# mala-lab/GGAD

Hardware: AMD Instinct MI355X
Metric: training nodes/sec (DGraph-Fin mini-batch GGAD) (higher is better)
Workload: dtype f32; 1 GPU; DGraph-Fin-size synthetic graph, mini-batch GGAD (GCN encoder); nodes=3700550, directed_entries=72953930, feat=17, emb=64, batch=150+50, graph=powerlaw(alpha=2.1,max_degree=2000), chunk_batches=150, hop2=ldsw, overlap=False, dense_cus=0, chain=0, dense_steps=XCD-resident chunk kernel: one launch per chunk on 28 CUs of one XCD, parallelism=dp1, optimizer=adam(lr=1e-3,wd=0.007), batch_streams=the reference's stream

## Files before the change

### ggad_amd/csrc/common.h

```cpp
#pragma once
#include <hip/hip_runtime.h>
#include <stdint.h>
#include <mutex>
#include "../../include/ggad_hip.h"

#define GGAD_WAVE 64
#define GGAD_MAX_D 64
#define GGAD_MAX_F 1024

void ggad_set_error(hipError_t e, const char *where);

#define GGAD_CHECK_LAUNCH(where)                 \
  do {                                           \
    hipError_t _e = hipGetLastError();           \
    if (_e != hipSuccess) {                      \
      ggad_set_error(_e, where);                 \
      return GGAD_E_LAUNCH;                      \
    }                                            \
  } while (0)

#define GGAD_REQUIRE(cond) \
  do {                     \
    if (!(cond)) return GGAD_E_INVALID; \
  } while (0)

static inline hipStream_t as_stream(ggad_stream_t s) { return reinterpret_cast<hipStream_t>(s); }

struct ggad_lds_optin {
  std::mutex mu;
  int state[64] = {};
};
template <typename... K>
static inline int ggad_lds_opt_in(ggad_lds_optin &S, int bytes, K... kernels) {
  int dev = 0;
  if (hipGetDevice(&dev) != hipSuccess || dev < 0 || dev >= 64) return 0;
  std::lock_guard<std::mutex> lock(S.mu);
  if (S.state[dev] == 0) {
    const bool ok = ((hipFuncSetAttribute((const void *)kernels, hipFuncAttributeMaxDynamicSharedMemorySize, bytes) == hipSuccess) && ...);
    (void)hipGetLastError();
    S.state[dev] = ok ? 1 : -1;
  }
  return S.state[dev];
}

__device__ __forceinline__ int lane_id() { return threadIdx.x & (GGAD_WAVE - 1); }

__device__ __forceinline__ float wave_sum(float v) {
#pragma unroll
  for (int off = 32; off >= 1; off >>= 1) v += __shfl_xor(v, off, GGAD_WAVE);
  return v;
}
__device__ __forceinline__ int wave_sum_i(int v) {
#pragma unroll
  for (int off = 32; off >= 1; off >>= 1) v += __shfl_xor(v, off, GGAD_WAVE);
  return v;
}

__device__ __forceinline__ void ggad_adam_elem(float &pi, float &mi, float &vi, float g, float wd, float sc0, float sc1) {
  float gi = fmaf(wd, pi, g);
  mi = fmaf(gi - mi, 0.1f, mi);
  vi = fmaf(0.001f * gi, gi, vi * 0.999f);
  const float denom = sqrtf(vi) / sc1 + 1e-8f;
  pi = pi - sc0 * (mi / denom);
}

__device__ __forceinline__ int lower_bound_i32(const int32_t *__restrict__ a, int lo, int hi, int key) {
  while (lo < hi) {
    int mid = (lo + hi) >> 1;
    if (a[mid] < key) lo = mid + 1; else hi = mid;
  }
  return lo;
}

__device__ __forceinline__ bool ggad_vblock(int skip, unsigned &vb, unsigned &vg) {
  const unsigned b = blockIdx.x, n = gridDim.x;
  if (skip < 0) { vb = b; vg = n; return true; }
  const unsigned sk = (unsigned)skip;
  if ((b & 7u) == sk) return false;
  vb = b - ((b >> 3) + ((b & 7u) > sk ? 1u : 0u));
  vg = n - ((n >> 3) + ((n & 7u) > sk ? 1u : 0u));
  return true;
}
static inline unsigned ggad_skip_grid(unsigned want, int skip) { return skip < 0 ? want : (unsigned)(((uint64_t)(want + 1) * 8 + 6) / 7); }

constexpr int GGAD_CTR_STRIDE = 16;
constexpr int GGAD_CTR_GROUPS = 0 * GGAD_CTR_STRIDE, GGAD_CTR_ITEMS = 1 * GGAD_CTR_STRIDE, GGAD_CTR_PART = 2 * GGAD_CTR_STRIDE,
              GGAD_CTR_CURSOR = 3 * GGAD_CTR_STRIDE, GGAD_CTR_PC = 4 * GGAD_CTR_STRIDE,
              GGAD_CTR_BIG = 5 * GGAD_CTR_STRIDE,
              GGAD_CTR_RANGE0 = 6 * GGAD_CTR_STRIDE,
              GGAD_CTR_PROF = 14 * GGAD_CTR_STRIDE;
constexpr int GGAD_RANGES = 8;
constexpr int GGAD_RANGE_DEG = 256;
constexpr int GGAD_PLAN_COUNTERS = 16 * GGAD_CTR_STRIDE;

struct ggad_plan_view {
  const int32_t *batch_ptr, *batch_ent_ptr, *nodes, *row_slot, *ent_ptr, *row_ck_ptr, *ck_rc, *ck_e0;
  int32_t n_batches, n_rows, n_ents, n_chunks;
  int32_t seg_stride;
  int64_t pair_bound;
};
int ggad_int_hop1(const ggad_mb_plan *P, const ggad_plan_view &V, int ldsw, int reset_now, hipStream_t st);
int ggad_int_global_hop2(const ggad_mb_plan *P, const ggad_plan_view &V, hipStream_t st, hipEvent_t ev0, hipEvent_t ev1);
int ggad_int_ldsw_hop2(const ggad_mb_plan *P, const ggad_plan_view &V, hipStream_t st, hipEvent_t ev0, hipEvent_t ev1);
int ggad_int_range_deg();

int ggad_int_gemm_slab(const float *A, const float *B, float *C, int M, int N, int K, int64_t lda, int64_t sbk, int64_t sbn, int64_t ldc,
                       const float *bias, int relu, hipStream_t st, const float *prelu_a = nullptr, float *C2 = nullptr, int64_t ldc2 = 0);

int64_t ggad_int_wgrad_tn_ws(int R, int m, int n);
int ggad_int_wgrad_tn(const float *P, int64_t ldp, const float *Q, int64_t ldq, int R, int m, int n, float *D, float *ws, hipStream_t st,
                      int *vpq = nullptr);

constexpr int GGAD_MB_BWD_PARTS = 256;
struct ggad_xchg_view;
bool ggad_int_wide_ok(int D, int F);
int ggad_int_wide_project(const float *params, int32_t D, int32_t F, const float *x2, const int32_t *ent_own, int32_t ent0,
                          int32_t n_ents, float *h2, ggad_stream_t stream);
int ggad_int_wide_fwd_rows(const float *params, int32_t D, int32_t F, const float *x1, const float *h2, const int32_t *ent_ptr,
                           const int32_t *ent_own, const int32_t *labels, int32_t row0, int32_t n_rows, int32_t ent0, float *h1,
                           float *nbar, float *gen, ggad_stream_t stream);
int ggad_int_wide_loss(const float *params, int32_t D, int32_t F, const float *h1, const float *nbar, const float *gen,
                       const int32_t *labels, const int32_t *pos_meta, const int32_t *row_pos, const int32_t *ent_ptr,
                       int32_t row0, int32_t n_rows, float *loss_ws, float *losses8, float *d_h1, float *d_gen, float *d_nbar,
                       float *dz, float *coef_a, float *coef_g, int32_t *step_counter, ggad_stream_t stream);
int ggad_int_wide_row_coefs(const float *params, int32_t D, int32_t F, const int32_t *labels, const int32_t *ent_ptr,
                            int32_t row0, int32_t n_rows, const float *h1, const float *gen, const float *d_h1,
                            const float *d_gen, const float *d_nbar, float *dz, float *coef_a, float *coef_g,
                            ggad_stream_t stream);
int ggad_int_wide_bwd_flat(int32_t D, int32_t F, const float *x1, const float *x2, const float *h2, const int32_t *ent_own,
                           const int32_t *ent_row, int32_t row0, int32_t n_rows, int32_t ent0, int32_t n_ents,
                           const float *coef_a, const float *coef_g, float *dw_part, ggad_stream_t stream);
int ggad_int_wide_grad_reduce(int32_t D, int32_t F, const int32_t *pos_meta, int32_t row0, int32_t n_rows, const float *losses8,
                              const float *nbar, const float *dw_part, const float *dz, const float *loss_ws, float *grads,
                              int mode, float *params, float *m, float *v, float lr, float wd, const int32_t *step_counter,
                              const ggad_xchg_view *xv, uint32_t xstep, float grad_scale, ggad_stream_t stream);
int ggad_int_wide_rows(const float *params, int32_t D, int32_t F, const float *x1, int32_t n_rows, float *out, int score,
                       ggad_stream_t stream);

constexpr int GGAD_XCHG_MAX_WORLD = 16;
struct ggad_xchg_view {
  float *peer[GGAD_XCHG_MAX_WORLD];
  int32_t rank, world;
  int64_t n;
  int32_t *err;
  unsigned long long timeout_ticks;
};
struct ggad_xchg {
  ggad_xchg_view view;
  void *local;
  size_t bytes;
  uint32_t step;
  bool opened[GGAD_XCHG_MAX_WORLD];
};
static inline size_t ggad_xchg_granules(int world, int64_t n) { return (size_t)2 * world * (size_t)n; }
```

### ggad_amd/csrc/hop2_ldsw.hip

```cpp
#include <algorithm>
#include <atomic>
#include <climits>
#include <mutex>

#include "common.h"

namespace {

#ifdef GGAD_G2_PROF
struct G2Prof { unsigned long long a[8], t; };
#define G2_ARG , G2Prof &prof
#define G2_PASS , prof
#define G2_MARK(i) do { __builtin_amdgcn_sched_barrier(0); __builtin_amdgcn_s_waitcnt(0); const unsigned long long t_ = wall_clock64(); \
                        prof.a[i] += t_ - prof.t; prof.t = t_; __builtin_amdgcn_sched_barrier(0); } while (0)
#define TC_MARK(i) do { __syncthreads(); if (threadIdx.x == 0) { const unsigned long long t_ = wall_clock64(); tcp[i] += t_ - tct; tct = t_; } } while (0)
#else
#define G2_ARG
#define G2_PASS
#define G2_MARK(i)
#define TC_MARK(i)
#endif

constexpr int SLICE = 256;
constexpr int GRP_W = 10;
constexpr int ITEM_GRAB = 4;

__global__ void __launch_bounds__(256) k_tile_offsets(const int32_t *__restrict__ rowptr, const int32_t *__restrict__ col,
                                                      int64_t n_nodes, int n_tiles, int shift, int32_t *__restrict__ off) {
  const int64_t u = (int64_t)blockIdx.x * blockDim.x + threadIdx.x;
  if (u >= n_nodes) return;
  const int s = rowptr[u], e = rowptr[u + 1];
  int32_t *o = off + u * (n_tiles + 1);
  int t = 0;
  for (int i = s; i < e; ++i) {
    const int tile = col[i] >> shift;
    while (t <= tile) { o[t] = i - s; ++t; }
  }
  while (t <= n_tiles) { o[t] = e - s; ++t; }
}

__global__ void __launch_bounds__(256) k_tm_blocksum(const int32_t *__restrict__ off, int64_t n_nodes, int n_tiles, int32_t *__restrict__ bsum) {
  __shared__ int wsum[4][64];
  const int lane = lane_id(), w = threadIdx.x >> 6;
  const int NT1 = n_tiles + 1;
  const int64_t u0 = (int64_t)blockIdx.x * 256 + 64 * w;
  for (int t0 = 0; t0 < n_tiles; t0 += 64) {
    const int t = t0 + lane;
    int acc = 0;
    if (t < n_tiles)
      for (int i = 0; i < 64 && u0 + i < n_nodes; ++i) { const int32_t *o = off + (u0 + i) * NT1 + t; acc += o[1] - o[0]; }
    wsum[w][lane] = acc;
    __syncthreads();
    if (w == 0 && t < n_tiles) bsum[(int64_t)blockIdx.x * n_tiles + t] = wsum[0][lane] + wsum[1][lane] + wsum[2][lane] + wsum[3][lane];
    __syncthreads();
  }
}

__global__ void __launch_bounds__(1024) k_tm_scan(int32_t *__restrict__ bsum, int64_t n_blocks, int n_tiles, int32_t *__restrict__ tile_base) {
  extern __shared__ int tot[];
  for (int t = threadIdx.x; t < n_tiles; t += blockDim.x) {
    int run = 0;
    int64_t b = 0;
    for (; b + 8 <= n_blocks; b += 8) {
      int v[8];
#pragma unroll
      for (int q = 0; q < 8; ++q) v[q] = bsum[(b + q) * n_tiles + t];
#pragma unroll
      for (int q = 0; q < 8; ++q) { bsum[(b + q) * n_tiles + t] = run; run += v[q]; }
    }
    for (; b < n_blocks; ++b) { const int v = bsum[b * n_tiles + t]; bsum[b * n_tiles + t] = run; run += v; }
    tot[t] = run;
  }
  __syncthreads();
  if (threadIdx.x == 0) {
    int run = 0;
    for (int t = 0; t < n_tiles; ++t) { tile_base[t] = run; run += tot[t]; }
    tile_base[n_tiles] = run;
  }
}

__global__ void __launch_bounds__(256) k_tm_fill(const int32_t *__restrict__ rowptr, const int32_t *__restrict__ col,
                                                 const int32_t *__restrict__ off, int64_t n_nodes, int n_tiles,
                                                 const int32_t *__restrict__ bsum, const int32_t *__restrict__ tile_base,
                                                 int32_t *__restrict__ tile_start, int32_t *__restrict__ col_t) {
  __shared__ int wsum[4][64];
  const int lane = lane_id(), w = threadIdx.x >> 6;
  const int NT1 = n_tiles + 1;
  const int64_t u0 = (int64_t)blockIdx.x * 256 + 64 * w;
  for (int t0 = 0; t0 <= n_tiles; t0 += 64) {
    const int t = t0 + lane;
    int acc = 0;
    if (t < n_tiles)
      for (int i = 0; i < 64 && u0 + i < n_nodes; ++i) { const int32_t *o = off + (u0 + i) * NT1 + t; acc += o[1] - o[0]; }
    wsum[w][lane] = acc;
    __syncthreads();
    if (t < n_tiles) {
      int pos = tile_base[t] + bsum[(int64_t)blockIdx.x * n_tiles + t];
      for (int ww = 0; ww < w; ++ww) pos += wsum[ww][lane];
      for (int i = 0; i < 64 && u0 + i < n_nodes; ++i) {
        const int64_t u = u0 + i;
        const int32_t *o = off + u * NT1 + t;
        const int o0 = o[0], o1 = o[1];
        tile_start[u * NT1 + t] = pos;
        const int32_t *src = col + rowptr[u] + o0;
        for (int j = 0; j < o1 - o0; ++j) col_t[pos + j] = src[j];
        pos += o1 - o0;
      }
    } else if (t == n_tiles) {
      for (int i = 0; i < 64 && u0 + i < n_nodes; ++i) tile_start[(u0 + i) * NT1 + t] = 0;
    }
    __syncthreads();
  }
}

constexpr int TW_SHIFT = 15;
constexpr int TW_TILE = 1 << TW_SHIFT;
constexpr int TW_MAXOWN = 6144;
constexpr int TW_T = 1024;
constexpr int TW_BRK = 1536;

constexpr int TT_SLAB = 128;
__global__ void __launch_bounds__(256) k_seg_transpose(const int32_t *__restrict__ tile_off, const int32_t *__restrict__ tile_start,
                                                       int n_tiles, const int32_t *__restrict__ ent_own,
                                                       const int32_t *__restrict__ ent_col, int n_ents, int64_t seg_stride,
                                                       int32_t *__restrict__ seg_t, int skip) {
  __shared__ int tl[TT_SLAB][65];
  unsigned vbx, vgx;
  if (!ggad_vblock(skip, vbx, vgx)) return;
  const int p0 = vbx * 64;
  if (p0 >= n_ents) return;
  const int lane = lane_id(), wid = threadIdx.x >> 6;
  const int NT1 = n_tiles + 1;
  int u_l = 0, own_l = 0;
  if (p0 + lane < n_ents) { own_l = ent_own[p0 + lane] == p0 + lane ? 1 : 0; u_l = own_l ? ent_col[p0 + lane] : 0; }
  for (int which = 0; which < (tile_start ? 2 : 1); ++which) {
  const int32_t *table = which ? tile_start : tile_off;
  int32_t *plane = seg_t + (which ? (int64_t)NT1 * seg_stride : 0);
  for (int t0 = 0; t0 < NT1; t0 += TT_SLAB) {
    int v0[16], v1[16];
    const int c0 = min(t0 + lane, NT1 - 1), c1 = min(t0 + 64 + lane, NT1 - 1);
#pragma unroll
    for (int jj = 0; jj < 16; ++jj) {
      const int j = wid + 4 * jj;
      const int u = __shfl(u_l, j, GGAD_WAVE);
      const int32_t *row = table + (int64_t)u * NT1;
      v0[jj] = row[c0];
      v1[jj] = row[c1];
    }
#pragma unroll
    for (int jj = 0; jj < 16; ++jj) {
      const int j = wid + 4 * jj;
      const int own = __shfl(own_l, j, GGAD_WAVE);
      if (t0 + lane < NT1) tl[lane][j] = own ? v0[jj] : 0;
      if (t0 + 64 + lane < NT1) tl[64 + lane][j] = own ? v1[jj] : 0;
    }
    __syncthreads();
    const int nt = min(TT_SLAB, NT1 - t0);
    for (int idx = threadIdx.x; idx < nt * 64; idx += 256) {
      const int tt = idx >> 6, j = idx & 63;
      if (p0 + j < n_ents) plane[(int64_t)(t0 + tt) * seg_stride + p0 + j] = tl[tt][j];
    }
    __syncthreads();
  }
  }
}

__device__ __forceinline__ int block_excl_scan_1024(int v, int *warp_buf, int *total) {
  const int lane = lane_id(), wid = threadIdx.x >> 6;
  int inc = v;
#pragma unroll
  for (int off = 1; off < 64; off <<= 1) {
    const int t = __shfl_up(inc, off, 64);
    if (lane >= off) inc += t;
  }
  if (lane == 63) warp_buf[wid] = inc;
  __syncthreads();
  int base = 0, tot = 0;
#pragma unroll
  for (int w = 0; w < 16; ++w) { const int sv = warp_buf[w]; if (w < wid) base += sv; tot += sv; }
  __syncthreads();
  *total = tot;
  return base + inc - v;
}

__global__ void __launch_bounds__(TW_T) k_tile_counts(const int32_t *__restrict__ col, const int32_t *__restrict__ seg_t,
                                                      int64_t n_cap, const int32_t *__restrict__ own_rp,
                                                      const int32_t *__restrict__ batch_ent_ptr,
                                                      const int32_t *__restrict__ pw_base, uint16_t *__restrict__ pc, int n_tiles,
                                                      int n_batches, int32_t *__restrict__ counters, int skip, int tile_major) {
  extern __shared__ __attribute__((aligned(16))) uint32_t lds_u[];
  uint32_t *cnt = lds_u;
  int *offs = reinterpret_cast<int *>(lds_u + TW_TILE / 2);
  int *segbeg = offs + TW_MAXOWN + 1;
  int *dst = segbeg + TW_MAXOWN;
  int *brk = dst + TW_MAXOWN;
  __shared__ int wbuf[16];
  unsigned vbx, vgx;
  if (!ggad_vblock(skip, vbx, vgx)) return;
  int t, b;
  const bool class_map = (tile_major & 2) != 0;
  tile_major &= 1;
  if (class_map) {
    const int nx = skip < 0 ? 8 : 7, c = (int)(blockIdx.x & 7u);
    const int ci = c - ((skip >= 0 && c > skip) ? 1 : 0);
    const unsigned j = blockIdx.x >> 3;
    const int nt_c = ci < n_tiles ? (n_tiles - ci + nx - 1) / nx : 0;
    if (j >= (unsigned)nt_c * (unsigned)n_batches) return;
    t = ci + nx * (int)(j / (unsigned)n_batches);
    b = (int)(j % (unsigned)n_batches);
  } else {
    if (vbx >= (unsigned)n_tiles * (unsigned)n_batches) return;
    t = (int)(vbx % (unsigned)n_tiles); b = (int)(vbx / (unsigned)n_tiles);
  }
  const int o0 = batch_ent_ptr[b], o1 = batch_ent_ptr[b + 1];
  const int n_own_all = o1 - o0;
  const int32_t *seg_lo = seg_t + (int64_t)t * n_cap, *seg_hi = seg_lo + n_cap;
  const int32_t *seg_st = tile_major ? seg_t + (int64_t)(n_tiles + 1 + t) * n_cap : own_rp;
#ifdef GGAD_G2_PROF
  unsigned long long tcp[8] = {0, 0, 0, 0, 0, 0, 0, 0}, tct = wall_clock64();
#endif
  for (int i = threadIdx.x; i < TW_TILE / 2; i += TW_T) cnt[i] = 0u;
  constexpr int IPT = TW_MAXOWN / TW_T;
  const int n_slabs = (n_own_all + TW_MAXOWN - 1) / TW_MAXOWN;
  const bool one_slab = n_slabs == 1;
  constexpr int CACHE_IT = 16;
  int kc[CACHE_IT], dc[CACHE_IT];
  for (int pass = 0; pass < 2; ++pass) {
    for (int slab = 0; slab < n_slabs; ++slab) {
      const int ob0 = o0 + slab * TW_MAXOWN;
      const int n_own = min(TW_MAXOWN, o1 - ob0);
      if (pass == 0 || n_slabs > 1) {
        {
          int lo_[IPT], hi_[IPT], rp_[IPT], pb_[IPT];
#pragma unroll
          for (int q = 0; q < IPT; ++q) {
            const int i = min((int)threadIdx.x + q * TW_T, n_own - 1);
            lo_[q] = seg_lo[ob0 + i]; hi_[q] = seg_hi[ob0 + i]; rp_[q] = seg_st[ob0 + i]; pb_[q] = pw_base[ob0 + i];
          }
#pragma unroll
          for (int q = 0; q < IPT; ++q) {
            const int i = (int)threadIdx.x + q * TW_T;
            if (i < n_own) { offs[i] = hi_[q] - lo_[q]; segbeg[i] = rp_[q] + (tile_major ? 0 : lo_[q]); dst[i] = pb_[q] + lo_[q]; }
          }
        }
        __syncthreads();
        TC_MARK(0);
        int len[IPT];
        int mysum = 0;
#pragma unroll
        for (int q = 0; q < IPT; ++q) {
          const int i = threadIdx.x * IPT + q;
          len[q] = (i < n_own) ? offs[i] : 0;
          mysum += len[q];
        }
        __syncthreads();
        int P0;
        int ex = block_excl_scan_1024(mysum, wbuf, &P0);
#pragma unroll
        for (int q = 0; q < IPT; ++q) {
          const int i = threadIdx.x * IPT + q;
          if (i < n_own) offs[i] = ex;
          ex += len[q];
        }
        if (threadIdx.x == 0) offs[n_own] = P0;
        __syncthreads();
        TC_MARK(1);
      }
      const int P = offs[n_own];
      if (P > 0) {
        const int s0 = 1 << (31 - __clz(n_own));
        auto locate = [&](int pp, int &own, int &j) {
          int lo = 0;
          for (int st = s0; st > 0; st >>= 1) { const int m = lo + st; lo = (offs[min(m, n_own)] <= pp) ? m : lo; }
          own = lo; j = pp - offs[lo];
        };
        const int nblk = ((P - 1) >> 6) + 1;
        const bool use_brk = nblk + 1 <= TW_BRK;
        if (use_brk && (pass == 0 || n_slabs > 1)) {
          for (int b = threadIdx.x; b <= nblk; b += TW_T) {
            int own = n_own, j = 0;
            if (b < nblk) locate(min(64 * b, P - 1), own, j);
            brk[b] = own;
          }
          __syncthreads();
        }
        auto locate4 = [&](const int (&pp)[4], int (&own)[4], int (&j)[4]) {
          int lo[4] = {0, 0, 0, 0};
          int smax = s0;
          if (use_brk) {
            smax = 0;
#pragma unroll
            for (int q = 0; q < 4; ++q) {
              const int b = pp[q] >> 6;
              lo[q] = brk[b];
              const int w = brk[b + 1] - lo[q];
              smax = max(smax, w > 0 ? 1 << (31 - __clz(w)) : 0);
            }
          }
          for (int st = smax; st > 0; st >>= 1) {
#pragma unroll
            for (int q = 0; q < 4; ++q) { const int m = lo[q] + st; lo[q] = (offs[min(m, n_own)] <= pp[q]) ? m : lo[q]; }
          }
#pragma unroll
          for (int q = 0; q < 4; ++q) { own[q] = lo[q]; j[q] = pp[q] - offs[lo[q]]; }
        };
        int p_start = 0;
        if (one_slab) {
          if (pass == 0) {
#pragma unroll
            for (int g4 = 0; g4 < CACHE_IT; g4 += 4) {
              if (g4 * TW_T < P) {
                int pp[4], own[4], j[4];
#pragma unroll
                for (int q = 0; q < 4; ++q) pp[q] = min((g4 + q) * TW_T + (int)threadIdx.x, P - 1);
                locate4(pp, own, j);
#pragma unroll
                for (int q = 0; q < 4; ++q) {
                  kc[g4 + q] = col[segbeg[own[q]] + j[q]];
                  dc[g4 + q] = dst[own[q]] + j[q];
                }
              } else {
#pragma unroll
                for (int q = 0; q < 4; ++q) { kc[g4 + q] = 0; dc[g4 + q] = 0; }
              }
            }
#pragma unroll
            for (int it = 0; it < CACHE_IT; ++it) {
              const bool on = it * TW_T + (int)threadIdx.x < P;
              const int loc = kc[it] & (TW_TILE - 1);
              if (on) atomicAdd(&cnt[loc >> 1], 1u << ((loc & 1) << 4));
              kc[it] = on ? loc : -1;
            }
          } else {
#pragma unroll
            for (int it = 0; it < CACHE_IT; ++it)
              if (kc[it] >= 0) pc[dc[it]] = (uint16_t)((cnt[kc[it] >> 1] >> ((kc[it] & 1) << 4)) & 0xFFFFu);
          }
          p_start = CACHE_IT * TW_T;
          TC_MARK(2 + 2 * pass);
        }
        for (int p0 = p_start; p0 < P; p0 += 4 * TW_T) {
          int pp[4], own[4], j[4];
#pragma unroll
          for (int q = 0; q < 4; ++q) pp[q] = min(p0 + q * TW_T + (int)threadIdx.x, P - 1);
          locate4(pp, own, j);
          int k4[4];
#pragma unroll
          for (int q = 0; q < 4; ++q) k4[q] = col[segbeg[own[q]] + j[q]];
#pragma unroll
          for (int q = 0; q < 4; ++q) {
            if (p0 + q * TW_T + (int)threadIdx.x < P) {
              const int loc = k4[q] & (TW_TILE - 1);
              if (pass == 0) atomicAdd(&cnt[loc >> 1], 1u << ((loc & 1) << 4));
              else pc[(int64_t)dst[own[q]] + j[q]] = (uint16_t)((cnt[loc >> 1] >> ((loc & 1) << 4)) & 0xFFFFu);
            }
          }
        }
        TC_MARK(3 + 2 * pass);
      }
      __syncthreads();
    }
  }
#ifdef GGAD_G2_PROF
  if (threadIdx.x == 0) {
    unsigned long long *out = reinterpret_cast<unsigned long long *>(counters + GGAD_CTR_PROF) + 8;
    for (int k = 0; k < 6; ++k) atomicAdd(out + k, tcp[k]);
    atomicAdd(out + 6, 1ull);
  }
#endif
}

template <int G, int FT>
__device__ __forceinline__ void gather_slice(const int32_t *__restrict__ col, const float *__restrict__ feat, int F_rt, int stride,
                                             int s, int n0, int n1, float inv_sr, int n_occ, const int (&pb)[8],
                                             const uint16_t *__restrict__ pc, int lane, int k_first, float (&tot)[G] G2_ARG) {
  const int F = FT ? FT : F_rt;
  const int rpi = 64 / F;
  const int g = lane / F, f = lane - g * F;
  const bool act = g < rpi;
  const int gl = act ? g : rpi - 1;
  const char *fb = reinterpret_cast<const char *>(feat);
  const uint32_t rs = (uint32_t)stride * 4u, fo = (uint32_t)f * 4u;
  auto row_elem = [&](int kk) -> float { return *reinterpret_cast<const float *>(fb + ((uint32_t)kk * rs + fo)); };
  float acc[G];
#pragma unroll
  for (int j = 0; j < G; ++j) acc[j] = 0.0f;
  const int last = max(n1 - 1, 0);
  int k_nx = k_first;
  uint32_t c_nx[G];
  {
    const int ix = min(n0 + lane, last);
#pragma unroll
    for (int j = 0; j < G; ++j) c_nx[j] = pc[pb[j] + ix];
  }
  G2_MARK(2);
  for (int blk = n0; blk < n1; blk += 64) {
    const bool mine = blk + lane < n1;
    const int k = mine ? k_nx : 0;
    const int count = min(64, n1 - blk);
    float w[G];
    if (FT != 17) {
#pragma unroll
      for (int j = 0; j < G; ++j) w[j] = (j < n_occ && mine) ? inv_sr / sqrtf((float)c_nx[j]) : 0.0f;
    }
    if (FT == 17) {
      constexpr int IT = 22;
      float x[IT];
#pragma unroll
      for (int t = 0; t < IT; ++t) {
        const int kk = __shfl(k, (t * 3 + gl) & 63, GGAD_WAVE);
        x[t] = row_elem(kk);
      }
#pragma unroll
      for (int j = 0; j < G; ++j) w[j] = (j < n_occ && mine) ? inv_sr / sqrtf((float)c_nx[j]) : 0.0f;
      {
        const int ix = min(blk + 64 + lane, last);
        k_nx = col[s + ix];
#pragma unroll
        for (int j = 0; j < G; ++j) c_nx[j] = pc[pb[j] + ix];
      }
      G2_MARK(3);
#pragma unroll
      for (int t = 0; t < IT; ++t) {
        const int src = t * 3 + g;
        const float xv = (act && src < count) ? x[t] : 0.0f;
#pragma unroll
        for (int j = 0; j < G; ++j) {
          const float ws = __shfl(w[j], src & 63, GGAD_WAVE);
          acc[j] = fmaf((src < count) ? ws : 0.0f, xv, acc[j]);
        }
      }
      G2_MARK(4);
    } else {
      const int iters = (count + rpi - 1) / rpi;
      int tt = 0;
      for (; tt + 8 <= iters; tt += 8) {
        float x[8];
#pragma unroll
        for (int q = 0; q < 8; ++q) {
          const int kk = __shfl(k, ((tt + q) * rpi + gl) & 63, GGAD_WAVE);
          x[q] = row_elem(kk);
        }
#pragma unroll
        for (int q = 0; q < 8; ++q) {
          const int src = (tt + q) * rpi + g;
          const float xv = (act && src < count) ? x[q] : 0.0f;
#pragma unroll
          for (int j = 0; j < G; ++j) {
            const float ws = __shfl(w[j], src & 63, GGAD_WAVE);
            acc[j] = fmaf((src < count) ? ws : 0.0f, xv, acc[j]);
          }
        }
      }
      for (; tt < iters; ++tt) {
        const int src = tt * rpi + g;
        const int kk = __shfl(k, (tt * rpi + gl) & 63, GGAD_WAVE);
        const float xr = row_elem(kk);
        const float xv = (act && src < count) ? xr : 0.0f;
#pragma unroll
        for (int j = 0; j < G; ++j) {
          const float ws = __shfl(w[j], src & 63, GGAD_WAVE);
          acc[j] = fmaf((src < count) ? ws : 0.0f, xv, acc[j]);
        }
      }
      const int ix = min(blk + 64 + lane, last);
      k_nx = col[s + ix];
#pragma unroll
      for (int j = 0; j < G; ++j) c_nx[j] = pc[pb[j] + ix];
    }
  }
#pragma unroll
  for (int j = 0; j < G; ++j) {
    float t = acc[j];
    for (int q = 1; q < rpi; ++q) t += __shfl(acc[j], (lane + q * F) & 63, GGAD_WAVE);
    tot[j] = t;
  }
}

constexpr int MF_WS = 68;
constexpr int MF_LDS = 8 * MF_WS + 64;
typedef float mf4 __attribute__((ext_vector_type(4)));
typedef float mf2 __attribute__((ext_vector_type(2)));
typedef int mi4 __attribute__((ext_vector_type(4)));

template <int G>
__device__ __forceinline__ void gather_slice_mfma(const int32_t *__restrict__ col, const float *__restrict__ feat, int s, int n0, int n1,
                                                  float inv_sr, int n_occ, const int (&pb)[8], const uint16_t *__restrict__ pc,
                                                  int lane, float *lw, int k_first, float (&tot)[G] G2_ARG) {
  const int a = lane & 15, g = lane >> 4;
  const char *fb = reinterpret_cast<const char *>(feat) + a * 8;
  int *lids = reinterpret_cast<int *>(lw + 8 * MF_WS);
  const int aa = a < G ? a : 0;
  mf4 acc0 = {0.0f, 0.0f, 0.0f, 0.0f}, acc1 = {0.0f, 0.0f, 0.0f, 0.0f};
  const int last = max(n1 - 1, 0);
  int k_nx = k_first;
  uint32_t c_nx[G];
  {
    const int ix = min(n0 + lane, last);
#pragma unroll
    for (int j = 0; j < G; ++j) c_nx[j] = pc[pb[j] + ix];
  }
  G2_MARK(2);
  for (int blk = n0; blk < n1; blk += 64) {
    const bool mine = blk + lane < n1;
    lids[lane] = k_nx;
    __builtin_amdgcn_fence(__ATOMIC_RELEASE, "wavefront");
    __builtin_amdgcn_wave_barrier();
    int id[16];
#pragma unroll
    for (int c = 0; c < 4; ++c) {
      const mi4 iv = *reinterpret_cast<const mi4 *>(lids + 16 * g + 4 * c);
#pragma unroll
      for (int q = 0; q < 4; ++q) id[4 * c + q] = iv[q];
    }
    mf2 x[16];
#pragma unroll
    for (int i = 0; i < 16; ++i) x[i] = *reinterpret_cast<const mf2 *>(fb + ((uint32_t)id[i] << 7));
#pragma unroll
    for (int j = 0; j < G; ++j)
      lw[j * MF_WS + lane] = (j < n_occ && mine) ? inv_sr / sqrtf((float)c_nx[j]) : 0.0f;
// ... 189 lines not shown
      int e[8], pb[8];
      int n = 0;
#pragma unroll
      for (int j = 0; j < 8; ++j) {
        e[j] = __builtin_amdgcn_readlane(rv, q * 16 + j);
        pb[j] = __builtin_amdgcn_readlane(pbv, q * 16 + j);
        n += e[j] >= 0 ? 1 : 0;
      }
      const int pbase = __builtin_amdgcn_readlane(rv, q * 16 + 8), ns = __builtin_amdgcn_readlane(rv, q * 16 + 9);
      const int sl = __builtin_amdgcn_readlane(iv, q * 16 + 1);
      int s, n0, n1, deg;
      item_span(q, s, n0, n1, deg);
      const float inv_sr = 1.0f / sqrtf((float)deg);
      const int k_first = k_ahead;
      if (q + 1 < ITEM_GRAB && base + q + 1 < last) {
        int s_, a_, b_, d_;
        item_span(q + 1, s_, a_, b_, d_);
        k_ahead = first_ids(s_, a_, b_);
      }
      float tot[8];
      if (MF) {
        if (n == 1) { float t1[1]; gather_slice_mfma<1>(col, feat, s, n0, n1, inv_sr, n, pb, pc, lane, lw, k_first, t1 G2_PASS); tot[0] = t1[0]; }
        else if (n == 2) { float t2[2]; gather_slice_mfma<2>(col, feat, s, n0, n1, inv_sr, n, pb, pc, lane, lw, k_first, t2 G2_PASS); tot[0] = t2[0]; tot[1] = t2[1]; }
        else if (n <= 4) { float t4[4]; gather_slice_mfma<4>(col, feat, s, n0, n1, inv_sr, n, pb, pc, lane, lw, k_first, t4 G2_PASS);
#pragma unroll
          for (int j = 0; j < 4; ++j) tot[j] = t4[j]; }
        else gather_slice_mfma<8>(col, feat, s, n0, n1, inv_sr, n, pb, pc, lane, lw, k_first, tot G2_PASS);
      } else
      if (n == 1) { float t1[1]; gather_slice<1, FT>(col, feat, F, stride, s, n0, n1, inv_sr, n, pb, pc, lane, k_first, t1 G2_PASS); tot[0] = t1[0]; }
      else if (n == 2) { float t2[2]; gather_slice<2, FT>(col, feat, F, stride, s, n0, n1, inv_sr, n, pb, pc, lane, k_first, t2 G2_PASS); tot[0] = t2[0]; tot[1] = t2[1]; }
      else if (n <= 4) { float t4[4]; gather_slice<4, FT>(col, feat, F, stride, s, n0, n1, inv_sr, n, pb, pc, lane, k_first, t4 G2_PASS);
#pragma unroll
        for (int j = 0; j < 4; ++j) tot[j] = t4[j]; }
      else gather_slice<8, FT>(col, feat, F, stride, s, n0, n1, inv_sr, n, pb, pc, lane, k_first, tot G2_PASS);
#pragma unroll
      for (int j = 0; j < 8; ++j) {
        if (j < n && lane < F) {
          if (ns == 1) x2[(int64_t)e[j] * F + lane] = (deg == 0) ? inv_sr * 0.0f : tot[j];
          else part2[((int64_t)pbase + (int64_t)j * ns + sl) * F + lane] = tot[j];
        }
      }
      G2_MARK(5);
    }
    }
  }
  }
#ifdef GGAD_G2_PROF
  if (lane == 0) {
    prof.a[6] = wall_clock64() - t_begin;
    unsigned long long *out = reinterpret_cast<unsigned long long *>(counters + GGAD_CTR_PROF);
    for (int k = 0; k < 7; ++k) atomicAdd(out + k, prof.a[k]);
  }
#endif
}

__global__ void __launch_bounds__(256) k_gather2_combine(const int32_t *__restrict__ grp, const int32_t *__restrict__ counters,
                                                         const float *__restrict__ part2, int F, float *__restrict__ x2, int skip) {
  unsigned vbx, vgx;
  if (!ggad_vblock(skip, vbx, vgx)) return;
  const int lane = lane_id();
  const int n_groups = counters[GGAD_CTR_GROUPS];
  const int rpi = 64 / F;
  const int g = lane / F, f = lane - g * F;
  for (int gi = vbx * 4 + (threadIdx.x >> 6); gi < n_groups; gi += vgx * 4) {
    const int rv = (lane < GRP_W) ? grp[(int64_t)gi * GRP_W + lane] : -1;
    const int ns = __builtin_amdgcn_readlane(rv, 9);
    if (ns <= 1) continue;
    const int pbase = __builtin_amdgcn_readlane(rv, 8);
    for (int j0 = 0; j0 < 8; j0 += rpi) {
      const int j = j0 + g;
      const int ej = __shfl(rv, j & 7, GGAD_WAVE);
      if (g < rpi && j < 8 && ej >= 0) {
        float acc = 0.0f;
#pragma unroll 4
        for (int sl = 0; sl < ns; ++sl) acc += part2[((int64_t)pbase + (int64_t)j * ns + sl) * F + f];
        x2[(int64_t)ej * F + f] = acc;
      }
    }
  }
}

__global__ void __launch_bounds__(256) k_gather2_w(const int32_t *__restrict__ col, const float *__restrict__ feat, int F, int stride,
                                                   const int32_t *__restrict__ ent_own, int n_ents,
                                                   const int32_t *__restrict__ own_rp, const int32_t *__restrict__ own_deg,
                                                   const int32_t *__restrict__ pw_base, const uint16_t *__restrict__ pc,
                                                   float *__restrict__ x2, int skip) {
  unsigned vbx, vgx;
  if (!ggad_vblock(skip, vbx, vgx)) return;
  const int e0 = vbx * 4 + (threadIdx.x >> 6);
  if (e0 >= n_ents || ent_own[e0] != e0) return;
  const int lane = lane_id();
  const int s = own_rp[e0];
  const int deg = own_deg[e0];
  const int pb0 = pw_base[e0];
  const float inv_sr = 1.0f / sqrtf((float)deg);
  if (F <= 64) {
    const int pb[8] = {pb0, 0, 0, 0, 0, 0, 0, 0};
    float total = 0.0f;
#ifdef GGAD_G2_PROF
    G2Prof prof = {};
#endif
    for (int n0 = 0; n0 < deg; n0 += SLICE) {
      float t1[1];
      const int kf = col[s + min(n0 + lane, max(min(deg, n0 + SLICE) - 1, 0))];
      if (F == 17) gather_slice<1, 17>(col, feat, F, stride, s, n0, min(deg, n0 + SLICE), inv_sr, 1, pb, pc, lane, kf, t1 G2_PASS);
      else gather_slice<1, 0>(col, feat, F, stride, s, n0, min(deg, n0 + SLICE), inv_sr, 1, pb, pc, lane, kf, t1 G2_PASS);
      total += t1[0];
    }
    if (deg == 0) total = inv_sr * 0.0f;
    if (lane < F) x2[(int64_t)e0 * F + lane] = total;
    return;
  }
  for (int fbase = 0; fbase < F; fbase += 64) {
    const int fw = min(64, F - fbase);
    float total = 0.0f;
    for (int n0 = 0; n0 < deg; n0 += SLICE) {
      const int n1 = min(deg, n0 + SLICE);
      float acc = 0.0f;
      for (int blk = n0; blk < n1; blk += 64) {
        const int idx = blk + lane;
        int k = 0;
        float w = 0.0f;
        if (idx < n1) { k = col[s + idx]; w = inv_sr / sqrtf((float)pc[pb0 + idx]); }
        const int count = min(64, n1 - blk);
        for (int t = 0; t < count; ++t) {
          const int kk = __shfl(k, t, GGAD_WAVE);
          const float ws = __shfl(w, t, GGAD_WAVE);
          const float x = lane < fw ? feat[(int64_t)kk * stride + fbase + lane] : 0.0f;
          acc = fmaf(ws, x, acc);
        }
      }
      total += acc;
    }
    if (deg == 0) total = inv_sr * 0.0f;
    if (lane < fw) x2[(int64_t)e0 * F + fbase + lane] = total;
  }
}

std::atomic<int> g_mfma_batches{[] { const char *e = getenv("GGAD_GATHER_MFMA_BATCHES"); return e ? atoi(e) : 0; }()};
std::atomic<int> g_range_deg{[] { const char *e = getenv("GGAD_RANGE_DEG"); return e ? atoi(e) : 0; }()};

}

int ggad_int_range_deg() { return g_range_deg.load() > 0 ? std::max(g_range_deg.load(), GGAD_RANGE_DEG) : INT32_MAX; }

int ggad_int_ldsw_hop2(const ggad_mb_plan *P, const ggad_plan_view &V, hipStream_t st, hipEvent_t ev0, hipEvent_t ev1) {
  if (V.n_ents == 0 || V.n_batches == 0) return GGAD_OK;
  const int n_tiles = (int)((P->n_nodes + TW_TILE - 1) >> TW_SHIFT);
  const int skip = P->xcd_skip >= 0 && P->xcd_skip < 8 ? P->xcd_skip : -1;
  const bool tile_major = P->tile_start != nullptr && P->col_t != nullptr;
  k_seg_transpose<<<dim3(ggad_skip_grid((unsigned)((V.n_ents + 63) / 64), skip)), dim3(256), 0, st>>>(
      P->tile_off, tile_major ? P->tile_start : nullptr, n_tiles, P->ent_own, P->ent_col, V.n_ents, V.seg_stride, P->seg_t, skip);
  const size_t lds = (size_t)(TW_TILE / 2) * 4 + (size_t)(3 * TW_MAXOWN + 1) * 4 + (size_t)TW_BRK * 4;
  {
    static std::mutex mu;
    static int state[64] = {};
    int dev = 0;
    if (hipGetDevice(&dev) != hipSuccess || dev < 0 || dev >= 64) return GGAD_E_INVALID;
    std::lock_guard<std::mutex> lock(mu);
    if (state[dev] == 0) {
      const bool ok = hipFuncSetAttribute((const void *)k_tile_counts, hipFuncAttributeMaxDynamicSharedMemorySize, (int)lds) == hipSuccess;
      (void)hipGetLastError();
      state[dev] = ok ? 1 : -1;
    }
    if (state[dev] != 1) { ggad_set_error(hipErrorInvalidValue, "mb_plan_build: this device cannot give k_tile_counts its LDS"); return GGAD_E_LAUNCH; }
  }
  if (P->ev_tile0) (void)hipEventRecord(static_cast<hipEvent_t>(P->ev_tile0), st);
  static const int tc_map = [] { const char *e = getenv("GGAD_TC_MAP"); return e ? atoi(e) : -1; }();
  const bool class_map = tc_map >= 0 ? tc_map != 0 : tile_major;
  const unsigned tc_grid = class_map ? 8u * (unsigned)((n_tiles + (skip < 0 ? 8 : 7) - 1) / (skip < 0 ? 8 : 7)) * (unsigned)V.n_batches
                                      : ggad_skip_grid((unsigned)n_tiles * (unsigned)V.n_batches, skip);
  k_tile_counts<<<dim3(tc_grid), dim3(TW_T), lds, st>>>(tile_major ? P->col_t : P->col, P->seg_t, V.seg_stride, P->own_rp, V.batch_ent_ptr,
                                                        P->pw_base, P->pc, n_tiles, V.n_batches, P->counters, skip, (tile_major ? 1 : 0) | (class_map ? 2 : 0));
  if (P->ev_tile1) (void)hipEventRecord(static_cast<hipEvent_t>(P->ev_tile1), st);
  if (ev0) (void)hipEventRecord(ev0, st);
  const int F = P->feat_dim;
  if (P->node_major && F <= 64) {
    const int range_deg = ggad_int_range_deg();
    static const int affine = [] { const char *e = getenv("GGAD_RANGE_AFFINE"); return e ? atoi(e) : 1; }();
    int32_t *big = P->items + 2 * (int64_t)P->item_cap, *gbnd = P->items + 3 * (int64_t)P->item_cap;
    k_build_groups<<<dim3(ggad_skip_grid((unsigned)((V.n_ents + 255) / 256), skip)), dim3(256), 0, st>>>(
        P->ent_own, P->ent_col, P->own_deg, V.n_ents, P->node_head, P->own_next, P->tile_off, n_tiles, P->grp, P->items, big, gbnd,
        P->counters, range_deg, skip);
    const int64_t max_items = (int64_t)V.n_ents + (V.pair_bound > 0 ? V.pair_bound : P->pair_cap) / SLICE;
    static const int env_wg = [] { const char *e = getenv("GGAD_G2_WG_PER_CU"); return e ? atoi(e) : 0; }();
    static const int env_cap = [] { const char *e = getenv("GGAD_G2_TAKE_CAP"); return e ? atoi(e) : 0; }();
    const bool small_launch = V.n_batches <= 32;
    const int wg_per_cu = env_wg > 0 ? env_wg : (small_launch ? 3 : 4);
    const int take_cap = env_cap > 0 ? env_cap : (small_launch ? 8 : 12);
    const unsigned wgs = (unsigned)std::min<int64_t>((max_items + 4 * ITEM_GRAB - 1) / (4 * ITEM_GRAB), 256 * wg_per_cu);
    if (F == 17 && P->feat_stride == 32 && V.n_batches >= g_mfma_batches.load())
      k_gather2_items<17, true><<<dim3(ggad_skip_grid(wgs, skip)), dim3(256), 0, st>>>(P->col, P->feat, F, P->feat_stride, P->own_rp, P->own_deg,
                                                                                       P->pw_base, P->pc, P->grp, P->items, big, gbnd, P->counters,
                                                                                       P->x2, P->part2, affine, take_cap, skip);
    else if (F == 17)
      k_gather2_items<17, false><<<dim3(ggad_skip_grid(wgs, skip)), dim3(256), 0, st>>>(P->col, P->feat, F, P->feat_stride, P->own_rp, P->own_deg,
                                                                                 P->pw_base, P->pc, P->grp, P->items, big, gbnd, P->counters,
                                                                                 P->x2, P->part2, affine, take_cap, skip);
    else
      k_gather2_items<0, false><<<dim3(ggad_skip_grid(wgs, skip)), dim3(256), 0, st>>>(P->col, P->feat, F, P->feat_stride, P->own_rp, P->own_deg,
                                                                                P->pw_base, P->pc, P->grp, P->items, big, gbnd, P->counters,
                                                                                P->x2, P->part2, affine, take_cap, skip);
    const unsigned cg = (unsigned)std::min<int64_t>(((int64_t)V.n_ents + 3) / 4, 16384);
    k_gather2_combine<<<dim3(ggad_skip_grid(cg, skip)), dim3(256), 0, st>>>(P->grp, P->counters, P->part2, F, P->x2, skip);
  } else {
    k_gather2_w<<<dim3(ggad_skip_grid((unsigned)((V.n_ents + 3) / 4), skip)), dim3(256), 0, st>>>(
        P->col, P->feat, F, P->feat_stride, P->ent_own, V.n_ents, P->own_rp, P->own_deg, P->pw_base, P->pc, P->x2, skip);
  }
  if (ev1) (void)hipEventRecord(ev1, st);
  GGAD_CHECK_LAUNCH("mb_plan_build (ldsw 2-hop)");
  return GGAD_OK;
}

extern "C" {

int ggad_mb_ldsw_tile_shift(void) { return TW_SHIFT; }
int ggad_mb_ldsw_max_owners(void) { return TW_MAXOWN; }
int32_t ggad_mb_slice_len(void) { return SLICE; }
int32_t ggad_mb_group_words(void) { return GRP_W; }
int ggad_mb_set_gather_options(int32_t mfma_min_batches, int32_t range_deg) {
  if (mfma_min_batches >= 0) g_mfma_batches.store(mfma_min_batches);
  if (range_deg >= 0) g_range_deg.store(range_deg);
  return GGAD_OK;
}
int32_t ggad_mb_item_words(void) { return 3 + GGAD_RANGES + 1; }
int32_t ggad_mb_plan_counter_elems(void) { return GGAD_PLAN_COUNTERS; }
int64_t ggad_mb_tile_offsets_elems(int64_t n_nodes, int32_t tile_shift) {
  return n_nodes * (((n_nodes + (1LL << tile_shift) - 1) >> tile_shift) + 1);
}
int64_t ggad_mb_ldsw_seg_elems(int64_t n_nodes, int64_t n_entries_cap) {
  return 2 * (((n_nodes + TW_TILE - 1) >> TW_SHIFT) + 1) * ((n_entries_cap + 63) / 64 * 64);
}

int ggad_mb_tile_offsets(const int32_t *rowptr, const int32_t *col, int64_t n_nodes, int32_t tile_shift, int32_t *tile_off,
                         ggad_stream_t stream) {
  GGAD_REQUIRE(rowptr && col && tile_off && n_nodes >= 0 && tile_shift >= 8 && tile_shift <= 24);
  if (n_nodes == 0) return GGAD_OK;
  const int n_tiles = (int)((n_nodes + (1LL << tile_shift) - 1) >> tile_shift);
  k_tile_offsets<<<dim3((unsigned)((n_nodes + 255) / 256)), dim3(256), 0, as_stream(stream)>>>(rowptr, col, n_nodes, n_tiles,
                                                                                               tile_shift, tile_off);
  GGAD_CHECK_LAUNCH("mb_tile_offsets");
  return GGAD_OK;
}


int64_t ggad_mb_tile_major_workspace_elems(int64_t n_nodes, int32_t tile_shift) {
  if (n_nodes < 0 || tile_shift < 8 || tile_shift > 24) return 0;
  const int64_t n_tiles = (n_nodes + (1LL << tile_shift) - 1) >> tile_shift;
  return ((n_nodes + 255) / 256) * n_tiles + n_tiles + 1;
}

int ggad_mb_tile_major(const int32_t *rowptr, const int32_t *col, int64_t n_nodes, int32_t tile_shift, const int32_t *tile_off,
                       int32_t *tile_start, int32_t *col_t, int32_t *workspace, ggad_stream_t stream) {
  GGAD_REQUIRE(rowptr && col && tile_off && tile_start && col_t && workspace && n_nodes >= 0 && tile_shift >= 8 && tile_shift <= 24);
  if (n_nodes == 0) return GGAD_OK;
  const int n_tiles = (int)((n_nodes + (1LL << tile_shift) - 1) >> tile_shift);
  const int64_t n_blocks = (n_nodes + 255) / 256;
  GGAD_REQUIRE(n_tiles <= 16384 && n_blocks < (1LL << 31));
  hipStream_t st = as_stream(stream);
  int32_t *bsum = workspace, *tile_base = workspace + n_blocks * n_tiles;
  k_tm_blocksum<<<dim3((unsigned)n_blocks), dim3(256), 0, st>>>(tile_off, n_nodes, n_tiles, bsum);
  k_tm_scan<<<dim3(1), dim3(1024), (size_t)n_tiles * sizeof(int), st>>>(bsum, n_blocks, n_tiles, tile_base);
  k_tm_fill<<<dim3((unsigned)n_blocks), dim3(256), 0, st>>>(rowptr, col, tile_off, n_nodes, n_tiles, bsum, tile_base, tile_start, col_t);
  GGAD_CHECK_LAUNCH("mb_tile_major");
  return GGAD_OK;
}

}
```

Before: 3.324 million nodes/s.

## Make k_tile_counts a persistent kernel with ticket scheduling and next-unit prefetch

Turns the per-(tile,batch) k_tile_counts launch into a persistent grid of about one workgroup per CU. Each workgroup claims further units through an atomic ticket counter, and it prefetches the next unit's segment tables and batch entry bounds while the current unit is still being scanned. The aim is to cut workgroup launch and ramp-up cost and hide global-load latency for the small per-unit tables. In exchange it adds a global atomic per unit and a more complex control flow. The new ticket counter slot must also be reset between launches, and the diff does not show where that happens.

Result: slower. 3.279 million nodes/s (-1.4%).

```diff
diff --git a/ggad_amd/csrc/common.h b/ggad_amd/csrc/common.h
--- a/ggad_amd/csrc/common.h
+++ b/ggad_amd/csrc/common.h
@@ -88,7 +88,8 @@
               GGAD_CTR_CURSOR = 3 * GGAD_CTR_STRIDE, GGAD_CTR_PC = 4 * GGAD_CTR_STRIDE,
               GGAD_CTR_BIG = 5 * GGAD_CTR_STRIDE,
               GGAD_CTR_RANGE0 = 6 * GGAD_CTR_STRIDE,
-              GGAD_CTR_PROF = 14 * GGAD_CTR_STRIDE;
+              GGAD_CTR_PROF = 14 * GGAD_CTR_STRIDE,
+              GGAD_CTR_TICKET = 15 * GGAD_CTR_STRIDE + 14;
 constexpr int GGAD_RANGES = 8;
 constexpr int GGAD_RANGE_DEG = 256;
 constexpr int GGAD_PLAN_COUNTERS = 16 * GGAD_CTR_STRIDE;
diff --git a/ggad_amd/csrc/hop2_ldsw.hip b/ggad_amd/csrc/hop2_ldsw.hip
--- a/ggad_amd/csrc/hop2_ldsw.hip
+++ b/ggad_amd/csrc/hop2_ldsw.hip
@@ -165,8 +165,8 @@
   }
 }
 
-__device__ __forceinline__ int block_excl_scan_1024(int v, int *warp_buf, int *total) {
-  const int lane = lane_id(), wid = threadIdx.x >> 6;
+__device__ __forceinline__ int block_excl_scan_1024(int v, int tid, int *warp_buf, int *total) {
+  const int lane = tid & (GGAD_WAVE - 1), wid = tid >> 6;
   int inc = v;
 #pragma unroll
   for (int off = 1; off < 64; off <<= 1) {
@@ -187,7 +187,8 @@
                                                       int64_t n_cap, const int32_t *__restrict__ own_rp,
                                                       const int32_t *__restrict__ batch_ent_ptr,
                                                       const int32_t *__restrict__ pw_base, uint16_t *__restrict__ pc, int n_tiles,
-                                                      int n_batches, int32_t *__restrict__ counters, int skip, int tile_major) {
+                                                      int n_batches, int32_t *__restrict__ counters, int skip, int tile_major,
+                                                      int persist) {
   extern __shared__ __attribute__((aligned(16))) uint32_t lds_u[];
   uint32_t *cnt = lds_u;
   int *offs = reinterpret_cast<int *>(lds_u + TW_TILE / 2);
@@ -195,77 +196,134 @@
   int *dst = segbeg + TW_MAXOWN;
   int *brk = dst + TW_MAXOWN;
   __shared__ int wbuf[16];
+  __shared__ unsigned s_next;
   unsigned vbx, vgx;
   if (!ggad_vblock(skip, vbx, vgx)) return;
-  int t, b;
+  unsigned tidx = threadIdx.x;
   const bool class_map = (tile_major & 2) != 0;
   tile_major &= 1;
-  if (class_map) {
-    const int nx = skip < 0 ? 8 : 7, c = (int)(blockIdx.x & 7u);
-    const int ci = c - ((skip >= 0 && c > skip) ? 1 : 0);
-    const unsigned j = blockIdx.x >> 3;
-    const int nt_c = ci < n_tiles ? (n_tiles - ci + nx - 1) / nx : 0;
-    if (j >= (unsigned)nt_c * (unsigned)n_batches) return;
-    t = ci + nx * (int)(j / (unsigned)n_batches);
-    b = (int)(j % (unsigned)n_batches);
-  } else {
-    if (vbx >= (unsigned)n_tiles * (unsigned)n_batches) return;
-    t = (int)(vbx % (unsigned)n_tiles); b = (int)(vbx / (unsigned)n_tiles);
-  }
-  const int o0 = batch_ent_ptr[b], o1 = batch_ent_ptr[b + 1];
+  const int nx = skip < 0 ? 8 : 7;
+  const unsigned n_units = class_map ? 8u * (unsigned)((n_tiles + nx - 1) / nx) * (unsigned)n_batches : (unsigned)n_tiles * (unsigned)n_batches;
+  auto decode = [&](unsigned un, int &tt, int &bb) -> bool {
+    if (un >= n_units) return false;
+    int nt = n_tiles, nb = n_batches;
+    asm volatile("" : "+s"(nt), "+s"(nb));
+    if (class_map) {
+      const int c = (int)(un & 7u);
+      if (skip >= 0 && c == skip) return false;
+      const int ci = c - ((skip >= 0 && c > skip) ? 1 : 0);
+      const unsigned j = un >> 3;
+      const int nt_c = ci < n_tiles ? (n_tiles - ci + nx - 1) / nx : 0;
+      if (j >= (unsigned)nt_c * (unsigned)nb) return false;
+      tt = ci + nx * (int)(j / (unsigned)nb);
+      bb = (int)(j % (unsigned)nb);
+    } else {
+      tt = (int)(un % (unsigned)nt); bb = (int)(un / (unsigned)nt);
+    }
+    return true;
+  };
+  constexpr int IPT = TW_MAXOWN / TW_T;
+  auto fresh_tid = [&]() -> int { unsigned v = tidx; asm volatile("" : "+v"(v)); return (int)(v & (unsigned)(TW_T - 1)); };
+  struct Tables { int lo[IPT], hi[IPT], rp[IPT], pb[IPT]; };
+  Tables nxt;
+  auto request_tables = [&](Tables &T, int tt, int ob0, int n_own) {
+    const int32_t *seg_lo = seg_t + (int64_t)tt * n_cap, *seg_hi = seg_lo + n_cap;
+    const int32_t *seg_st = tile_major ? seg_t + (int64_t)(n_tiles + 1 + tt) * n_cap : own_rp;
+#pragma unroll
+    for (int q = 0; q < IPT; ++q) {
+      const int i = min((int)tidx + q * TW_T, n_own - 1);
+      T.lo[q] = seg_lo[ob0 + i]; T.hi[q] = seg_hi[ob0 + i]; T.rp[q] = seg_st[ob0 + i]; T.pb[q] = pw_base[ob0 + i];
+    }
+  };
+  auto tables_to_lds = [&](const Tables &T, int n_own) {
+    const int tl = fresh_tid();
+#pragma unroll
+    for (int q = 0; q < IPT; ++q) {
+      const int i = tl + q * TW_T;
+      if (i < n_own) { offs[i] = T.hi[q] - T.lo[q]; segbeg[i] = T.rp[q] + (tile_major ? 0 : T.lo[q]); dst[i] = T.pb[q] + T.lo[q]; }
+    }
+  };
+  auto request_ents = [&](bool ok, int bb) -> int { return batch_ent_ptr[(ok ? bb : 0) + (fresh_tid() & 1)]; };
+  const unsigned u_base = class_map ? gridDim.x : vgx;
+  unsigned u = class_map ? blockIdx.x : vbx;
+  if (u >= n_units) return;
+  int t = 0, o0, o1;
+  {
+    int b = 0;
+    const bool ok = decode(u, t, b);
+    const int ev = request_ents(ok, b);
+    o0 = __builtin_amdgcn_readlane(ev, 0); o1 = ok ? __builtin_amdgcn_readlane(ev, 1) : o0;
+    if (o1 > o0) request_tables(nxt, t, o0, min(TW_MAXOWN, o1 - o0));
+  }
+#ifdef GGAD_G2_PROF
+  unsigned long long tcp[8] = {0, 0, 0, 0, 0, 0, 0, 0}, tct = wall_clock64(), tc_units = 0;
+#endif
+  constexpr int CACHE_IT = 16;
+  static_assert(CACHE_IT % 2 == 0 && TW_SHIFT <= 15, "two tile-local ids per register");
+  unsigned kp[CACHE_IT / 2];
+  int dc[CACHE_IT];
+  while (u < n_units) {
+  asm volatile("" : "+v"(tidx));
+  tidx &= (unsigned)(TW_T - 1);
   const int n_own_all = o1 - o0;
-  const int32_t *seg_lo = seg_t + (int64_t)t * n_cap, *seg_hi = seg_lo + n_cap;
-  const int32_t *seg_st = tile_major ? seg_t + (int64_t)(n_tiles + 1 + t) * n_cap : own_rp;
-#ifdef GGAD_G2_PROF
-  unsigned long long tcp[8] = {0, 0, 0, 0, 0, 0, 0, 0}, tct = wall_clock64();
-#endif
-  for (int i = threadIdx.x; i < TW_TILE / 2; i += TW_T) cnt[i] = 0u;
-  constexpr int IPT = TW_MAXOWN / TW_T;
+  unsigned u_nx = n_units;
+  int t_nx = 0, b_nx = 0, ev_nx = 0, o0_nx = 0, o1_nx = 0;
+  bool ok_nx = false;
+  auto peek_next = [&]() {
+    u_nx = s_next;
+    ok_nx = decode(u_nx, t_nx, b_nx);
+    ev_nx = request_ents(ok_nx, b_nx);
+  };
+  auto prefetch_next = [&]() {
+    o0_nx = __builtin_amdgcn_readlane(ev_nx, 0); o1_nx = ok_nx ? __builtin_amdgcn_readlane(ev_nx, 1) : o0_nx;
+    if (o1_nx > o0_nx) request_tables(nxt, t_nx, o0_nx, min(TW_MAXOWN, o1_nx - o0_nx));
+  };
+  auto scan_slab = [&](int n_own, bool with_next) __attribute__((always_inline)) {
+    __syncthreads();
+    TC_MARK(0);
+    if (with_next) peek_next();
+    int len[IPT];
+    int mysum = 0;
+    const int ts = fresh_tid();
+#pragma unroll
+    for (int q = 0; q < IPT; ++q) {
+      const int i = ts * IPT + q;
+      len[q] = (i < n_own) ? offs[i] : 0;
+      mysum += len[q];
+    }
+    __syncthreads();
+    int P0;
+    int ex = block_excl_scan_1024(mysum, ts, wbuf, &P0);
+#pragma unroll
+    for (int q = 0; q < IPT; ++q) {
+      const int i = ts * IPT + q;
+      if (i < n_own) offs[i] = ex;
+      ex += len[q];
+    }
+    if (tidx == 0) offs[n_own] = P0;
+    __syncthreads();
+    TC_MARK(1);
+  };
+  unsigned ticket = 0;
+  if (persist && tidx == 0) ticket = atomicInc(reinterpret_cast<unsigned *>(&counters[GGAD_CTR_TICKET]), 0xFFFFFFFFu);
+  if (n_own_all > 0) tables_to_lds(nxt, min(TW_MAXOWN, n_own_all));
+  for (int i = tidx; i < TW_TILE / 2; i += TW_T) cnt[i] = 0u;
+  if (tidx == 0) s_next = persist ? u_base + ticket : n_units;
   const int n_slabs = (n_own_all + TW_MAXOWN - 1) / TW_MAXOWN;
   const bool one_slab = n_slabs == 1;
-  constexpr int CACHE_IT = 16;
-  int kc[CACHE_IT], dc[CACHE_IT];
   for (int pass = 0; pass < 2; ++pass) {
     for (int slab = 0; slab < n_slabs; ++slab) {
       const int ob0 = o0 + slab * TW_MAXOWN;
       const int n_own = min(TW_MAXOWN, o1 - ob0);
+      const bool first = pass == 0 && slab == 0;
       if (pass == 0 || n_slabs > 1) {
-        {
-          int lo_[IPT], hi_[IPT], rp_[IPT], pb_[IPT];
-#pragma unroll
-          for (int q = 0; q < IPT; ++q) {
-            const int i = min((int)threadIdx.x + q * TW_T, n_own - 1);
-            lo_[q] = seg_lo[ob0 + i]; hi_[q] = seg_hi[ob0 + i]; rp_[q] = seg_st[ob0 + i]; pb_[q] = pw_base[ob0 + i];
-          }
-#pragma unroll
-          for (int q = 0; q < IPT; ++q) {
-            const int i = (int)threadIdx.x + q * TW_T;
-            if (i < n_own) { offs[i] = hi_[q] - lo_[q]; segbeg[i] = rp_[q] + (tile_major ? 0 : lo_[q]); dst[i] = pb_[q] + lo_[q]; }
-          }
+        if (!first) {
+          request_tables(nxt, t, ob0, n_own);
+          tables_to_lds(nxt, n_own);
         }
-        __syncthreads();
-        TC_MARK(0);
-        int len[IPT];
-        int mysum = 0;
-#pragma unroll
-        for (int q = 0; q < IPT; ++q) {
-          const int i = threadIdx.x * IPT + q;
-          len[q] = (i < n_own) ? offs[i] : 0;
-          mysum += len[q];
-        }
-        __syncthreads();
-        int P0;
-        int ex = block_excl_scan_1024(mysum, wbuf, &P0);
-#pragma unroll
-        for (int q = 0; q < IPT; ++q) {
-          const int i = threadIdx.x * IPT + q;
-          if (i < n_own) offs[i] = ex;
-          ex += len[q];
-        }
-        if (threadIdx.x == 0) offs[n_own] = P0;
-        __syncthreads();
-        TC_MARK(1);
-      }
+        if (first) scan_slab(n_own, true); else scan_slab(n_own, false);
+      }
+      if (first && one_slab) prefetch_next();
       const int P = offs[n_own];
       if (P > 0) {
         const int s0 = 1 << (31 - __clz(n_own));
@@ -277,7 +335,7 @@
         const int nblk = ((P - 1) >> 6) + 1;
         const bool use_brk = nblk + 1 <= TW_BRK;
         if (use_brk && (pass == 0 || n_slabs > 1)) {
-          for (int b = threadIdx.x; b <= nblk; b += TW_T) {
+          for (int b = tidx; b <= nblk; b += TW_T) {
             int own = n_own, j = 0;
             if (b < nblk) locate(min(64 * b, P - 1), own, j);
             brk[b] = own;
@@ -307,12 +365,13 @@
         int p_start = 0;
         if (one_slab) {
           if (pass == 0) {
+            int kc[CACHE_IT];
 #pragma unroll
             for (int g4 = 0; g4 < CACHE_IT; g4 += 4) {
               if (g4 * TW_T < P) {
                 int pp[4], own[4], j[4];
 #pragma unroll
-                for (int q = 0; q < 4; ++q) pp[q] = min((g4 + q) * TW_T + (int)threadIdx.x, P - 1);
+                for (int q = 0; q < 4; ++q) pp[q] = min((g4 + q) * TW_T + (int)tidx, P - 1);
                 locate4(pp, own, j);
 #pragma unroll
                 for (int q = 0; q < 4; ++q) {
@@ -326,15 +385,18 @@
             }
 #pragma unroll
             for (int it = 0; it < CACHE_IT; ++it) {
-              const bool on = it * TW_T + (int)threadIdx.x < P;
+              const bool on = (int)tidx < P - it * TW_T;
               const int loc = kc[it] & (TW_TILE - 1);
               if (on) atomicAdd(&cnt[loc >> 1], 1u << ((loc & 1) << 4));
-              kc[it] = on ? loc : -1;
+              const unsigned h = on ? (unsigned)loc : 0xFFFFu;
+              kp[it >> 1] = (it & 1) ? (kp[it >> 1] | (h << 16)) : h;
             }
           } else {
 #pragma unroll
-            for (int it = 0; it < CACHE_IT; ++it)
-              if (kc[it] >= 0) pc[dc[it]] = (uint16_t)((cnt[kc[it] >> 1] >> ((kc[it] & 1) << 4)) & 0xFFFFu);
+            for (int it = 0; it < CACHE_IT; ++it) {
+              const unsigned h = (kp[it >> 1] >> ((it & 1) << 4)) & 0xFFFFu;
+              if (h != 0xFFFFu) pc[dc[it]] = (uint16_t)((cnt[h >> 1] >> ((h & 1u) << 4)) & 0xFFFFu);
+            }
           }
           p_start = CACHE_IT * TW_T;
           TC_MARK(2 + 2 * pass);
@@ -342,14 +404,14 @@
         for (int p0 = p_start; p0 < P; p0 += 4 * TW_T) {
           int pp[4], own[4], j[4];
 #pragma unroll
-          for (int q = 0; q < 4; ++q) pp[q] = min(p0 + q * TW_T + (int)threadIdx.x, P - 1);
+          for (int q = 0; q < 4; ++q) pp[q] = min(p0 + q * TW_T + (int)tidx, P - 1);
           locate4(pp, own, j);
           int k4[4];
 #pragma unroll
           for (int q = 0; q < 4; ++q) k4[q] = col[segbeg[own[q]] + j[q]];
 #pragma unroll
           for (int q = 0; q < 4; ++q) {
-            if (p0 + q * TW_T + (int)threadIdx.x < P) {
+            if ((int)tidx < P - p0 - q * TW_T) {
               const int loc = k4[q] & (TW_TILE - 1);
               if (pass == 0) atomicAdd(&cnt[loc >> 1], 1u << ((loc & 1) << 4));
               else pc[(int64_t)dst[own[q]] + j[q]] = (uint16_t)((cnt[loc >> 1] >> ((loc & 1) << 4)) & 0xFFFFu);
@@ -361,11 +423,22 @@
       __syncthreads();
     }
   }
+  if (n_slabs == 0) {
+    __syncthreads();
+    peek_next();
+    __syncthreads();
+  }
+  if (!one_slab) prefetch_next();
 #ifdef GGAD_G2_PROF
-  if (threadIdx.x == 0) {
+  ++tc_units;
+#endif
+  u = u_nx; t = t_nx; o0 = o0_nx; o1 = o1_nx;
+  }
+#ifdef GGAD_G2_PROF
+  if (tidx == 0) {
     unsigned long long *out = reinterpret_cast<unsigned long long *>(counters + GGAD_CTR_PROF) + 8;
     for (int k = 0; k < 6; ++k) atomicAdd(out + k, tcp[k]);
-    atomicAdd(out + 6, 1ull);
+    atomicAdd(out + 6, tc_units);
   }
 #endif
 }
@@ -861,26 +934,35 @@
   k_seg_transpose<<<dim3(ggad_skip_grid((unsigned)((V.n_ents + 63) / 64), skip)), dim3(256), 0, st>>>(
       P->tile_off, tile_major ? P->tile_start : nullptr, n_tiles, P->ent_own, P->ent_col, V.n_ents, V.seg_stride, P->seg_t, skip);
   const size_t lds = (size_t)(TW_TILE / 2) * 4 + (size_t)(3 * TW_MAXOWN + 1) * 4 + (size_t)TW_BRK * 4;
+  int n_cus = 256;
   {
     static std::mutex mu;
-    static int state[64] = {};
+    static int state[64] = {}, cus[64] = {};
     int dev = 0;
     if (hipGetDevice(&dev) != hipSuccess || dev < 0 || dev >= 64) return GGAD_E_INVALID;
     std::lock_guard<std::mutex> lock(mu);
     if (state[dev] == 0) {
       const bool ok = hipFuncSetAttribute((const void *)k_tile_counts, hipFuncAttributeMaxDynamicSharedMemorySize, (int)lds) == hipSuccess;
       (void)hipGetLastError();
+      if (hipDeviceGetAttribute(&cus[dev], hipDeviceAttributeMultiprocessorCount, dev) != hipSuccess || cus[dev] <= 0) cus[dev] = 256;
       state[dev] = ok ? 1 : -1;
     }
+    n_cus = cus[dev];
     if (state[dev] != 1) { ggad_set_error(hipErrorInvalidValue, "mb_plan_build: this device cannot give k_tile_counts its LDS"); return GGAD_E_LAUNCH; }
   }
   if (P->ev_tile0) (void)hipEventRecord(static_cast<hipEvent_t>(P->ev_tile0), st);
   static const int tc_map = [] { const char *e = getenv("GGAD_TC_MAP"); return e ? atoi(e) : -1; }();
   const bool class_map = tc_map >= 0 ? tc_map != 0 : tile_major;
-  const unsigned tc_grid = class_map ? 8u * (unsigned)((n_tiles + (skip < 0 ? 8 : 7) - 1) / (skip < 0 ? 8 : 7)) * (unsigned)V.n_batches
-                                      : ggad_skip_grid((unsigned)n_tiles * (unsigned)V.n_batches, skip);
+  const unsigned tc_units = class_map ? 8u * (unsigned)((n_tiles + (skip < 0 ? 8 : 7) - 1) / (skip < 0 ? 8 : 7)) * (unsigned)V.n_batches
+                                       : ggad_skip_grid((unsigned)n_tiles * (unsigned)V.n_batches, skip);
+  static const int tc_persist = [] { const char *e = getenv("GGAD_TC_PERSIST"); return e ? atoi(e) : 1; }();
+  static const int tc_env_wgs = [] { const char *e = getenv("GGAD_TC_WGS"); return e ? atoi(e) : 0; }();
+  const unsigned tc_want = tc_env_wgs > 0 ? (unsigned)tc_env_wgs : (unsigned)n_cus * (skip < 0 ? 8u : 7u) / 8u;
+  const unsigned tc_wgs = class_map ? (tc_want + 7u) / 8u * 8u : ggad_skip_grid(tc_want, skip);
+  const unsigned tc_grid = tc_persist ? std::min(tc_units, std::max(tc_wgs, 1u)) : tc_units;
   k_tile_counts<<<dim3(tc_grid), dim3(TW_T), lds, st>>>(tile_major ? P->col_t : P->col, P->seg_t, V.seg_stride, P->own_rp, V.batch_ent_ptr,
-                                                        P->pw_base, P->pc, n_tiles, V.n_batches, P->counters, skip, (tile_major ? 1 : 0) | (class_map ? 2 : 0));
+                                                        P->pw_base, P->pc, n_tiles, V.n_batches, P->counters, skip,
+                                                        (tile_major ? 1 : 0) | (class_map ? 2 : 0), tc_persist ? 1 : 0);
   if (P->ev_tile1) (void)hipEventRecord(static_cast<hipEvent_t>(P->ev_tile1), st);
   if (ev0) (void)hipEventRecord(ev0, st);
   const int F = P->feat_dim;
```
